# yandooo/cilium

Hardware: AMD Instinct MI355X
Metric: L7 verdicts/sec + scanned GB/s (HBM roofline frac), 1/2/4/8 MI355X (higher is better)
Workload: dtype u8

## Files before the change

### cilium_amd/csrc/capi.cc

```cpp
#include <algorithm>
#include <cstring>

#include "engine/nfa_pool.h"
#include "engine_state.h"
#include "policy/npds_proto.h"
#include "regex/nfa_walk.h"
#include "regex/re_dfa.h"

namespace {

void set_err(char *err, size_t errlen, const std::string &m) {
    if (!err || errlen == 0) return;
    size_t n = std::min(errlen - 1, m.size());
    memcpy(err, m.data(), n);
    err[n] = 0;
}

template <class T>
size_t Put(std::vector<uint8_t> &blob, const std::vector<T> &v) {
    size_t off = (blob.size() + 255) & ~(size_t)255;
    blob.resize(off + v.size() * sizeof(T) + 16);
    if (!v.empty()) memcpy(blob.data() + off, v.data(), v.size() * sizeof(T));
    return off;
}
// ... 246 lines not shown
    e->mc = std::make_unique<McCompiler>(e->ps.get());
    e->r2 = std::make_unique<R2Compiler>(e->ps.get());
    e->cs = std::make_unique<CassCompiler>(e->ps.get());
    return e;
}

void l7g_engine_destroy(l7g_engine *e) {
    if (!e) return;
    if (e->device < 0) { delete e; return; }
    hipSetDevice(e->device);
    StopServices(e);
    hipDeviceSynchronize();
    if (e->d_blob) hipFree(e->d_blob);
    if (e->d_conns) hipFree(e->d_conns);
    e->hctx.clear();
    e->scr.clear();
    if (e->d_flow) hipFree(e->d_flow);
    if (e->d_zreg) hipFree(e->d_zreg);
    if (e->zreg_ev) hipEventDestroy(e->zreg_ev);
    for (hipEvent_t ev : e->prof_ev)
        if (ev) hipEventDestroy(ev);
    delete e;
}

int l7g_policy_update(l7g_engine *e, const char *json, size_t len, char *err, size_t errlen) {
    return l7g_policy_update_view(e, (const uint8_t *)json, len, 0, 0, err, errlen);
}

int l7g_policy_update_proto(l7g_engine *e, const uint8_t *buf, size_t len, char *err, size_t errlen) {
    return l7g_policy_update_view(e, buf, len, 1, 0, err, errlen);
}

constexpr uint64_t kTablesMagic = 0x3154473754L;
constexpr uint64_t kTablesAbi = 2ull << 56 | (uint64_t)sizeof(DevRuleset) << 48 | (uint64_t)sizeof(DevNfa) << 36 |
                                (uint64_t)sizeof(ImgHeader) << 24 | (uint64_t)sizeof(DevKafkaRuleset) << 12 |
                                (uint64_t)sizeof(McImgHeader);

int l7g_tables_export(l7g_engine *e, uint8_t *buf, size_t cap, size_t *len) {
    std::lock_guard<std::mutex> g(e->mu);
    Ser s;
    s.u64(kTablesMagic);
    s.u64(kTablesAbi);
    s.u64((uint64_t)e->policy_form);
    s.u64((uint64_t)e->policy_px);
    s.str(e->policy_src);
    e->hc->Save(s);
    e->kc->Save(s);
    e->mc->Save(s);
    e->r2->Save(s);
    e->cs->Save(s);
    if (len) *len = s.out.size();
    if (!buf || cap < s.out.size()) return -2;
    memcpy(buf, s.out.data(), s.out.size());
    return 0;
}

int l7g_tables_import(l7g_engine *e, const uint8_t *buf, size_t len, char *err, size_t errlen) {
    std::lock_guard<std::mutex> g(e->mu);
    Des d(buf, len);
    if (d.u64() != kTablesMagic) { set_err(err, errlen, "not an l7g_tables_export image"); return -1; }
    if (d.u64() != kTablesAbi) { set_err(err, errlen, "tables image from a build with another table layout"); return -1; }
    const int form = (int)d.u64(), px = (int)d.u64();
    const std::string src = d.str();
    if (!d.ok) { set_err(err, errlen, "truncated tables image"); return -1; }
    auto ps = std::make_unique<PolicySet>();
    std::string m;
    const bool ok = form ? LoadPolicySetProto((const uint8_t *)src.data(), src.size(), ps.get(), &m)
// ... 218 lines not shown
```

### cilium_amd/csrc/device_tables.h

```cpp
#pragma once
#include <stddef.h>
#include <stdint.h>

#if defined(__HIPCC__)
#define L7_HD __host__ __device__
#else
#define L7_HD
#endif

namespace l7 {

enum : uint8_t {
    V_DENY = 0, V_ALLOW = 1, V_PARSE_ERROR = 2, V_INCOMPLETE = 3, V_UNSUPPORTED = 4,
};
enum : uint8_t { PROTO_NONE = 0, PROTO_HTTP = 1, PROTO_KAFKA = 2, PROTO_MEMCACHE = 3, PROTO_R2D2 = 4, PROTO_CASSANDRA = 5 };
#define L7_PROTO_OWNED(p) ((p) >= PROTO_HTTP && (p) <= PROTO_CASSANDRA)

#ifndef L7_KAFKA_CLASSES
#define L7_KAFKA_CLASSES 8
#endif

constexpr int kCntWords = 32;
constexpr int kCntMc = L7_KAFKA_CLASSES;
constexpr int kCntHttp = L7_KAFKA_CLASSES + 2;
// ... 55 lines not shown
    uint16_t len;
    uint16_t pad;
    uint32_t name_off;
};
struct ImgHeader {
    uint8_t nchunks;
    uint8_t nhdr;
    uint8_t terminal;
    uint8_t ndfa;
    uint8_t slot_dfa[kNumSlots + 1];
    uint8_t max_slot_dfas;
    uint8_t pad0[3];
    uint16_t ref_slots;
    uint16_t pad1;
    uint32_t dfa_off;
    uint32_t init_off;
    uint32_t absent_off;
    uint32_t rule_off;
    uint32_t hdr_off;
    uint32_t total_states;
    uint32_t name_cls_off;
    uint32_t name_trans_off;
    uint32_t name_info_off;
    uint16_t name_ncls;
    uint16_t name_states;
    uint32_t nfa_off;
    uint8_t nnfa;
    uint8_t ntab_bits;
    uint8_t pad2[2];
    uint32_t ntab_off;
    uint32_t ntab_mul;
};
static_assert(sizeof(ImgHeader) == 80, "ImgHeader layout");

struct DevNameEnt {
    uint32_t w[4];
    uint8_t len;
    uint8_t info;
    uint8_t pad[10];
};
L7_HD inline uint32_t l7_name_hash(uint32_t w0, uint32_t w1, uint32_t w2, uint32_t w3, uint32_t len, uint32_t mul,
                                   uint32_t bits) {
    uint32_t x = w0 ^ (w1 * 0x85EBCA6Bu) ^ (w2 * 0xC2B2AE35u) ^ (w3 * 0x27D4EB2Fu) ^ len;
    x ^= x >> 15;
    return (x * mul) >> (32 - bits);
}

constexpr int kNfaMaxWords = 16;
constexpr int kNfaMaxPositions = 1 << 20;
struct DevNfaSparse {
    uint64_t row_of_off;
    uint64_t row_ptr_off;
    uint64_t pair_w_off;
    uint64_t pair_m_off;
};
struct DevNfa {
    uint32_t m, W, K, nivl;
    uint64_t t_off;
    uint64_t ivl_off;
    uint64_t b_off;
    uint64_t acc_off;
    uint64_t ascii_off;
    uint8_t condmap[64];
};
constexpr int kMaxNfaPerRuleset = 64;
struct DevNfaRef {
// ... 176 lines not shown
```

### cilium_amd/csrc/engine/http_compile.cc

```cpp
#include "http_compile.h"

#include <algorithm>
#include <cstring>
#include <functional>
#include <memory>

#include "../regex/re_dfa.h"
#include "nfa_pool.h"

namespace l7 {

namespace {

constexpr int kSlotNever = 0xFF;
int FixedSlot(const std::string &name) {
    if (name == ":method") return SLOT_METHOD;
    if (name == ":path") return SLOT_PATH;
    if (name == ":authority") return SLOT_AUTHORITY;
    if (name == "host" || name == "x-envoy-original-dst-host") return kSlotNever;
    if (!name.empty() && name[0] == ':') return kSlotNever;
    return -1;
}

struct Pat {
// ... 377 lines not shown
                    if (rp.second == nf.pat && (a == 1) == pats[rp.second].invert) m[rp.first >> 6] &= ~bit(rp.first);
            }
        }
        H.max_slot_dfas = (uint8_t)std::max<size_t>(H.max_slot_dfas, dfas.size());
        for (size_t g = 0; g < dfas.size(); g++) {
            Built b{slot, std::move(dfas[g]), {}, 0};
            b.absorb = SortAbsorbing(b.d);
            const std::vector<int> &sub = groups[g];
            std::vector<int> local(pats.size(), -1);
            for (size_t q = 0; q < sub.size(); q++) local[sub[q]] = (int)q;
            b.masks.resize((size_t)b.d.nstates * nchunks);
            for (int s = 0; s < b.d.nstates; s++) {
                uint64_t *m = &b.masks[(size_t)s * nchunks];
                for (size_t c = 0; c < nchunks; c++) m[c] = all[c];
                for (auto &rp : rm_pat) {
                    int q = local[rp.second];
                    if (q < 0) continue;
                    bool acc = (b.d.accept[s][q >> 6] >> (q & 63)) & 1;
                    if (acc == pats[rp.second].invert) m[rp.first >> 6] &= ~bit(rp.first);
                }
            }
            built.push_back(std::move(b));
        }
    }
    if (built.size() > 255) { *err = "rule set needs more than 255 DFAs"; return -1; }
    if (nfas.size() > (size_t)kMaxNfaPerRuleset) { *err = "rule set needs more than 64 NFA matchers"; return -1; }
    H.nnfa = (uint8_t)nfas.size();
    H.ndfa = (uint8_t)built.size();
    for (int s = 0, k = 0; s <= kNumSlots; s++) {
        while (k < (int)built.size() && built[k].slot < s) k++;
        H.slot_dfa[s] = (uint8_t)k;
    }

    std::vector<uint8_t> img(sizeof(ImgHeader));
    std::vector<DevDfa> dd(built.size());
    H.dfa_off = Append(img, dd.data(), dd.size());
    H.init_off = Append(img, init.data(), init.size());
    H.absent_off = Append(img, absent.data(), absent.size());
    std::vector<int32_t> ids(nchunks * 64, -1);
    for (size_t r = 0; r < nr; r++) ids[r] = rules[r]->id;
    H.rule_off = Append(img, ids.data(), ids.size());
    std::vector<DevHdrName> hn;
    std::vector<uint8_t> names;
    for (auto &nm : custom) {
        DevHdrName h{};
        uint32_t hash = kFnvBasis;
        for (char c : nm) hash = l7_fnv_step(hash, (uint8_t)c);
        h.hash = hash;
        h.len = (uint16_t)nm.size();
        h.name_off = (uint32_t)names.size();
        names.insert(names.end(), nm.begin(), nm.end());
        hn.push_back(h);
    }
    {
        std::vector<DevNfaRef> refs(nfas.size());
        for (size_t k = 0; k < nfas.size(); k++) {
            refs[k].nfa = nfas[k].nfa;
            refs[k].slot = (uint8_t)nfas[k].slot;
            refs[k].mask_off = Append(img, nfas[k].masks.data(), nfas[k].masks.size());
        }
        H.nfa_off = Append(img, refs.data(), refs.size());
    }
    H.hdr_off = Append(img, hn.data(), hn.size());
    uint32_t names_off = Append(img, names.data(), names.size());
    for (auto &h : hn) h.name_off += names_off;
    if (!hn.empty()) memcpy(img.data() + H.hdr_off, hn.data(), hn.size() * sizeof(DevHdrName));
    {
        NameDfa nd = BuildNameDfa(custom);
        H.name_ncls = (uint16_t)nd.ncls;
        H.name_states = (uint16_t)nd.info.size();
        H.name_cls_off = Append(img, nd.cls, 256);
        H.name_trans_off = Append(img, nd.trans.data(), nd.trans.size());
        H.name_info_off = Append(img, nd.info.data(), nd.info.size());
        uint32_t bits = 0, mul = 0;
        const std::vector<DevNameEnt> tab = BuildNameTable(custom, &bits, &mul);
        H.ntab_bits = (uint8_t)bits;
        H.ntab_mul = mul;
        H.ntab_off = Append(img, tab.data(), tab.size());
    }
    for (size_t k = 0; k < built.size(); k++) {
        const re::DFA &d = built[k].d;
        dd[k].ncls = (uint16_t)d.ncls;
        dd[k].start = (uint16_t)d.start;
        dd[k].cls_off = Append(img, d.cls, 256);
        dd[k].trans_off = Append(img, d.next.data(), d.next.size());
        dd[k].mask_off = Append(img, built[k].masks.data(), built[k].masks.size());
        dd[k].absorb = built[k].absorb;
        H.total_states += (uint32_t)d.nstates;
    }
    memcpy(img.data() + H.dfa_off, dd.data(), dd.size() * sizeof(DevDfa));
    memcpy(img.data(), &H, sizeof H);
    img.resize((img.size() + 15) & ~(size_t)15);

    HttpImage &I = img_;
    DevRuleset rs{};
    rs.image_off = (uint32_t)I.images.size();
    rs.image_len = (uint32_t)img.size();
    if ((uint64_t)rs.image_off + img.size() > 0xFFFFFFFFull) { *err = "HTTP rule tables exceed 4 GiB"; return -1; }
    I.images.insert(I.images.end(), img.begin(), img.end());
    I.rulesets.push_back(rs);
    I.chunks += nchunks;
    I.dfas += built.size();
    I.dfa_states += H.total_states;
    return (int)I.rulesets.size() - 1;
}

}
```

### cilium_amd/csrc/kernels/http_classify.hip

```cpp
#include <hip/hip_runtime.h>

#include <algorithm>
#include <cstddef>

#include "../device_tables.h"
#include "copy_in.h"
#include "gmem.h"
#include "launch.h"
#include "service.h"

extern "C" __device__ __attribute__((const)) unsigned long long __ockl_wfred_min_u64(unsigned long long);
extern "C" __device__ __attribute__((const)) unsigned long long __ockl_wfred_max_u64(unsigned long long);
extern "C" __device__ __attribute__((const)) unsigned long long __ockl_wfred_and_u64(unsigned long long);

namespace l7 {

namespace {

constexpr int kWaves = 8;
constexpr int kBlock = 64 * kWaves;
constexpr uint32_t kWin = 256;
constexpr uint32_t kWinChunks = kWin / 16;
constexpr uint32_t kWaveLds = 64 * kWin;
constexpr uint32_t kOffImg = kWaves * kWaveLds;
// ... 11 lines not shown
#define PH_DECL uint64_t ph_t = __builtin_amdgcn_s_memtime(); uint64_t ph_acc[8] = {0, 0, 0, 0, 0, 0, 0, 0};
#define PH_MARK(slot) do { const uint64_t ph_n = __builtin_amdgcn_s_memtime(); ph_acc[slot] += ph_n - ph_t; ph_t = ph_n; } while (0)
#define PH_COUNT(slot, v) (ph_acc[slot] += (v))
#define PH_FLUSH(lane) do { if ((lane) == 0) for (int ph_i = 0; ph_i < 8; ph_i++) atomicAdd(&g_phase[ph_i], (unsigned long long)ph_acc[ph_i]); } while (0)
#else
#define PH_DECL
#define PH_MARK(slot) do {} while (0)
#define PH_COUNT(slot, v) do {} while (0)
#define PH_FLUSH(lane) do {} while (0)
#endif
#ifdef L7G_PHASE_TIMING
#define LAT_T0 uint64_t lat_t = __builtin_amdgcn_s_memtime();
#define LAT_T(slot) do { const uint64_t lat_n = __builtin_amdgcn_s_memtime(); if ((threadIdx.x & 63) == 0) atomicAdd(&g_phase[slot], (unsigned long long)(lat_n - lat_t)); lat_t = lat_n; } while (0)
#define LAT_N(slot) do { if ((threadIdx.x & 63) == 0) atomicAdd(&g_phase[slot], 1ull); } while (0)
#else
#define LAT_T0
#define LAT_T(slot) do {} while (0)
#define LAT_N(slot) do {} while (0)
#endif

enum : uint32_t {
    M_METHOD, M_TARGET, M_VERSION, M_LINE, M_NAME, M_OWS, M_VALUE, M_SKIP, M_LF, M_ENDLF, M_DONE,
    M_CHSIZE, M_CHEXT, M_CHLF, M_CHDATA, M_CHDCR, M_CHDLF, M_TRL, M_TRLSCAN, M_TRLLF, M_TRLEND
};
constexpr uint32_t kNoSlot = 0xFF;

__constant__ uint32_t kVer[10] = {'H', 'T', 'T', 'P', '/', 0x100, '.', 0x100, '\r', '\n'};

__device__ __forceinline__ bool is_tchar(uint32_t c) {
    const uint32_t m1 = 0x03FF6CFAu;
    const uint32_t m2 = 0xC7FFFFFEu;
    const uint32_t m3 = 0x57FFFFFFu;
    const uint32_t w = c < 0x40 ? m1 : (c < 0x60 ? m2 : m3);
    return (c - 0x20u < 0x60u) && ((w >> (c & 31)) & 1);
}

__device__ __forceinline__ uint32_t stop_bits(uint32_t x) {
    const uint32_t t = x & 0x7F7F7F7Fu;
    return (~(t + 0x60606060u) | (t + 0x01010101u)) & ~x & 0x80808080u;
}
__device__ __forceinline__ uint32_t nib(uint32_t s) { return __builtin_amdgcn_ubfe((s >> 7) * 0x204081u, 21, 4); }
__device__ __forceinline__ uint32_t stop_mask(uint4 w) {
    return nib(stop_bits(w.x)) | nib(stop_bits(w.y)) << 4 | nib(stop_bits(w.z)) << 8 | nib(stop_bits(w.w)) << 12;
}
__device__ __forceinline__ uint32_t tstop_bits(uint32_t x) {
    const uint32_t t = x & 0x7F7F7F7Fu;
    return (~(t + 0x5F5F5F5Fu) | (t + 0x01010101u)) & ~x & 0x80808080u;
}
__device__ __forceinline__ uint32_t vstop_bits(uint32_t x) {
    const uint32_t t = x ^ 0x09090909u;
    const uint32_t ht = ~(((t & 0x7F7F7F7Fu) + 0x7F7F7F7Fu) | t) & 0x80808080u;
    return stop_bits(x) & ~ht;
}
__device__ __forceinline__ uint32_t stop_any(uint4 w) {
    const uint32_t a = w.x & 0x7F7F7F7Fu, b = w.y & 0x7F7F7F7Fu, c = w.z & 0x7F7F7F7Fu, d = w.w & 0x7F7F7F7Fu;
    const uint32_t s = ((~(a + 0x60606060u) | (a + 0x01010101u)) & ~w.x) | ((~(b + 0x60606060u) | (b + 0x01010101u)) & ~w.y) |
                       ((~(c + 0x60606060u) | (c + 0x01010101u)) & ~w.z) | ((~(d + 0x60606060u) | (d + 0x01010101u)) & ~w.w);
    return s & 0x80808080u;
}
__device__ __forceinline__ uint32_t alnum_bits(uint32_t x) {
    const uint32_t h = x | 0x80808080u;
    const uint32_t l = x | 0xA0A0A0A0u;
    const uint32_t dig = (h - 0x30303030u) & ~(h - 0x3A3A3A3Au);
    const uint32_t let = (l - 0x61616161u) & ~(l - 0x7B7B7B7Bu);
    const uint32_t t = x ^ 0x2D2D2D2Du;
    const uint32_t dash = ~(((t & 0x7F7F7F7Fu) + 0x7F7F7F7Fu) | t);
    return (dig | let | dash) & ~x & 0x80808080u;
}
// ... 23 lines not shown
    __device__ __forceinline__ uint4 u128(uint32_t o) const { return *(const uint4 *)(p + o); }
};
template <bool kLds>
__device__ __forceinline__ uint32_t uni(uint32_t v) {
    return kLds ? (uint32_t)__builtin_amdgcn_readfirstlane((int)v) : v;
}
#define HDR_U32(I, field) uni<kLds>((I).u32(offsetof(ImgHeader, field)))
#define HDR_U16(I, field) uni<kLds>((I).u16(offsetof(ImgHeader, field)))
#define HDR_U8(I, field) uni<kLds>((I).u8(offsetof(ImgHeader, field)))

struct Lane {
    uint64_t base;
    uint32_t a0;
    uint32_t lena;
    uint32_t pa;
    uint32_t w;
    uint32_t mode;
    uint32_t mark;
    uint32_t idx;
    bool done;
    bool owed;
    bool scan;
    bool tail;
    uint8_t verdict;
    int32_t rule;
    uint32_t consumed;
    uint32_t present;
    uint32_t slot;
    uint32_t nstate;
    uint32_t ninfo;
    bool have_cl, chunked, cl_bad, cl_ws, in_ows;
    uint32_t ndig;
    uint64_t clv, cl;
    uint32_t dcls, dtrans, dmask, dncls, st, saved;
    uint32_t dabs;
    uint64_t acc[kChunksPerPass];
    uint32_t cg, dg;
};
static_assert(kDfasPerPass == 1, "one DFA per slot per framing pass");

template <bool kLds>
__device__ __forceinline__ void slot_begin(const Img<kLds> &I, Lane &L, uint32_t slot) {
    const uint32_t lo = I.u8(offsetof(ImgHeader, slot_dfa) + slot) + L.dg;
    const uint32_t hi = I.u8(offsetof(ImgHeader, slot_dfa) + slot + 1);
    L.st = 0;
    L.dcls = L.dtrans = L.dmask = L.dncls = L.dabs = 0;
    if (lo < hi) {
        const uint32_t d = HDR_U32(I, dfa_off) + lo * sizeof(DevDfa);
        L.dcls = I.u32(d + 0);
        L.dtrans = I.u32(d + 4);
        L.dmask = I.u32(d + 8);
        const uint32_t nc_st = I.u32(d + 12);
        L.dncls = nc_st & 0xFFFF;
        L.st = nc_st >> 16;
        L.dabs = I.u32(d + 16);
    }
}

template <bool kLds>
__device__ __forceinline__ void dfa_step(const Img<kLds> &I, Lane &L, uint32_t c) {
    if (L.st) L.st = I.u16(L.dtrans + 2 * (L.st * L.dncls + I.u8(L.dcls + c)));
}

template <bool kLds>
__device__ __forceinline__ void slot_end(const Img<kLds> &I, Lane &L) {
    if (L.dtrans == 0) return;
    const uint32_t nchunks = HDR_U8(I, nchunks);
    const uint32_t nc = nchunks > L.cg ? min(nchunks - L.cg, (uint32_t)kChunksPerPass) : 0;
    const uint32_t base = L.dmask + 8 * (L.st * nchunks + L.cg);
#pragma unroll
    for (int c = 0; c < kChunksPerPass; c++)
        if ((uint32_t)c < nc) L.acc[c] &= I.u64(base + 8 * c);
}

template <bool kLds>
__device__ __forceinline__ void acc_init(const Img<kLds> &I, Lane &L) {
    const uint32_t nchunks = HDR_U8(I, nchunks);
#pragma unroll
    for (int c = 0; c < kChunksPerPass; c++)
        L.acc[c] = L.cg + c < nchunks ? I.u64(HDR_U32(I, init_off) + 8 * (L.cg + c)) : 0;
}

template <bool kLds>
__device__ __forceinline__ void frame_reset(const Img<kLds> &I, Lane &L) {
    L.pa = L.a0;
    L.mode = M_METHOD;
    L.mark = L.a0;
    L.present = 0;
    L.have_cl = L.chunked = false;
    L.cl = 0;
    slot_begin(I, L, SLOT_METHOD);
}

__device__ __forceinline__ void finish(Lane &L, uint8_t v, int32_t rule = -1) {
    L.done = true;
    L.scan = false;
    L.mode = M_DONE;
    L.verdict = v;
    L.rule = rule;
// ... 64 lines not shown
            } else {
                verdict_then_body(L, (uint8_t)HDR_U8(I, terminal), -1);
            }
        }
    }
}

template <bool kLds>
__device__ __forceinline__ bool line_done(const Img<kLds> &I, Lane &L) {
    bool ok = true;
    if (L.ninfo & NI_CL) {
        ok = !(L.have_cl || L.ndig == 0 || L.ndig > 10 || L.cl_bad);
        L.have_cl = true;
        L.cl = L.clv;
    }
    if ((L.ninfo & NI_TE) && L.ndig == 7) L.chunked = true;
    if (L.slot != kNoSlot) {
        slot_end(I, L);
        L.present |= 1u << L.slot;
    }
    return ok;
}

struct Cursor {
    const uint8_t *slot;
    uint32_t swz;
    uint32_t w;
    __device__ __forceinline__ uint4 chunk(uint32_t k) const {
        return *(const uint4 *)(slot + (((k << 4) & (kWin - 16)) ^ swz));
    }
    __device__ __forceinline__ uint32_t at(uint32_t p) const { return slot[((p - w) & (kWin - 1)) ^ swz]; }
};

template <int kKind>
__device__ __forceinline__ uint32_t find_stop(const Cursor &C, uint32_t pa, uint32_t lim) {
    while (pa < lim) {
        const uint4 w = C.chunk((pa - C.w) >> 4);
        uint32_t m = (kKind == 0 ? tstop_mask(w) : kKind == 1 ? vstop_mask(w) : nonalnum_mask(w)) & (0xFFFFu << (pa & 15));
        const uint32_t cend = (pa & ~15u) + 16;
        if (cend > lim) m &= (1u << (lim & 15)) - 1u;
        if (m) return (pa & ~15u) + (uint32_t)__builtin_ctz(m);
        pa = cend;
    }
    return lim;
}

template <bool kLds>
__device__ __forceinline__ void ows_done(const Img<kLds> &I, Lane &L) {
    if (L.slot == kNoSlot && !(L.ninfo & (NI_CL | NI_TE))) {
        L.mode = M_SKIP;
    } else {
        L.mode = M_VALUE;
        if (L.slot != kNoSlot) {
            slot_begin(I, L, L.slot);
        } else {
            L.st = 0;
            L.dcls = L.dtrans = 0;
        }
        L.in_ows = false;
        L.clv = 0;
        L.ndig = 0;
        L.cl_bad = L.cl_ws = false;
    }
}

template <bool kLds>
__device__ __forceinline__ void name_slot(const Img<kLds> &I, Lane &L) {
    uint32_t s = kNoSlot;
    if (L.ninfo & NI_HOST) s = SLOT_AUTHORITY;
    else if (L.ninfo & NI_CUSTOM) s = SLOT_CUSTOM0 + (L.ninfo & NI_CUSTOM) - 1;
    if (s != kNoSlot && ((L.present >> s) & 1)) s = kNoSlot;
    if (s != kNoSlot && !((HDR_U32(I, ref_slots) >> s) & 1)) s = kNoSlot;
    L.slot = s;
}

__device__ __forceinline__ uint32_t ws_mask(uint4 w) {
    auto eq = [](uint32_t x, uint32_t b) {
        const uint32_t t = x ^ b;
        return ~(((t & 0x7F7F7F7Fu) + 0x7F7F7F7Fu) | t) & 0x80808080u;
    };
    return nib(eq(w.x, 0x20202020u) | eq(w.x, 0x09090909u)) | nib(eq(w.y, 0x20202020u) | eq(w.y, 0x09090909u)) << 4 |
           nib(eq(w.z, 0x20202020u) | eq(w.z, 0x09090909u)) << 8 | nib(eq(w.w, 0x20202020u) | eq(w.w, 0x09090909u)) << 12;
}

template <bool kLds>
__device__ __forceinline__ void fast_line(const Img<kLds> &I, Lane &L, const Cursor &C, const uint64_t *nfa_bits) {
    const uint32_t k0 = (L.pa - C.w) >> 4, o = L.pa & 15, i = o >> 2, sh = (o & 3) * 8;
    const uint4 a = C.chunk(k0), b = C.chunk(k0 + 1);
    const uint32_t d1 = i == 0 ? a.y : i == 1 ? a.z : i == 2 ? a.w : b.x;
    const uint32_t d0 = i == 0 ? a.x : i == 1 ? a.y : i == 2 ? a.z : a.w;
// ... 21 lines not shown
    if (nb == 0) return;
    auto keep = [e](uint32_t j) { return e >= 4 * j + 4 ? 0xFFFFFFFFu : e <= 4 * j ? 0u : (1u << (8 * (e - 4 * j))) - 1u; };
    const uint32_t w0 = (f.x | 0x20202020u) & keep(0), w1 = (f.y | 0x20202020u) & keep(1);
    const uint32_t w2 = (f.z | 0x20202020u) & keep(2), w3 = (f.w | 0x20202020u) & keep(3);
    const uint32_t h = l7_name_hash(w0, w1, w2, w3, e, HDR_U32(I, ntab_mul), nb);
    const uint32_t ent = HDR_U32(I, ntab_off) + h * (uint32_t)sizeof(DevNameEnt);
    const uint4 n = I.u128(ent);
    const uint32_t meta = I.u32(ent + 16);
    const bool hit = (meta & 0xFF) == e && n.x == w0 && n.y == w1 && n.z == w2 && n.w == w3;
    L.mark = L.pa;
    L.ninfo = hit ? (meta >> 8) & 0xFF : 0u;
    name_slot(I, L);
    const uint32_t v = (uint32_t)__builtin_ctz((~ws_mask(f) & (0xFFFFu << (e + 1)) & 0xFFFFu) | 0x10000u);
    if (v < 16) {
        L.pa += v;
        ows_done(I, L);
    } else {
        L.pa += e + 1;
        L.mode = M_OWS;
    }
}

template <bool kLds>
__device__ __forceinline__ void parse_window(const Img<kLds> &I, Lane &L, Cursor &C, const uint64_t *nfa_bits) {
    const uint32_t lim = min(L.w + kWin, L.lena);
    C.w = L.w;
    const uint32_t ncls_name = HDR_U16(I, name_ncls);
    const uint32_t name_cls = HDR_U32(I, name_cls_off), name_trans = HDR_U32(I, name_trans_off);

    if (L.mode == M_METHOD) {
        uint32_t c = 0;
        if (L.pa < lim) {
            c = C.at(L.pa);
            uint32_t k = L.dcls ? I.u8(L.dcls + c) : 0;
            uint32_t c1 = L.pa + 1 < lim ? C.at(L.pa + 1) : 0;
            while (is_tchar(c)) {
                const uint32_t p1 = L.pa + 1;
                const uint32_t c2 = p1 + 1 < lim ? C.at(p1 + 1) : 0;
                const uint32_t k1 = L.dcls ? I.u8(L.dcls + c1) : 0;
                if (L.st) L.st = I.u16(L.dtrans + 2 * (L.st * L.dncls + k));
                L.pa = p1;
                if (p1 >= lim) break;
                c = c1;
                c1 = c2;
                k = k1;
            }
        }
        if (L.pa < lim) {
            if (c != ' ' || L.pa == L.mark) {
                finish(L, V_PARSE_ERROR);
            } else {
                slot_end(I, L);
                L.present |= 1u << SLOT_METHOD;
                L.pa++;
                L.mark = L.pa;
                L.mode = M_TARGET;
                slot_begin(I, L, SLOT_PATH);
            }
        }
    }
    if (L.mode == M_TARGET) {
        uint32_t c = 0;
        if (L.pa < lim) {
            c = C.at(L.pa);
            uint32_t k = L.dcls ? I.u8(L.dcls + c) : 0;
            uint32_t c1 = L.pa + 1 < lim ? C.at(L.pa + 1) : 0;
            while (c > 0x20 && c != 0x7F && L.st != 0 && L.st < L.dabs) {
                const uint32_t p1 = L.pa + 1;
                const uint32_t c2 = p1 + 1 < lim ? C.at(p1 + 1) : 0;
                const uint32_t k1 = L.dcls ? I.u8(L.dcls + c1) : 0;
                if (L.st) L.st = I.u16(L.dtrans + 2 * (L.st * L.dncls + k));
                L.pa = p1;
                if (p1 >= lim) break;
                c = c1;
                c1 = c2;
                k = k1;
            }
        }
        if (L.pa < lim && c > 0x20 && c != 0x7F) {
            L.pa = find_stop<0>(C, L.pa, lim);
            c = L.pa < lim ? C.at(L.pa) : 0;
        }
        if (L.pa < lim) {
            if (c != ' ' || L.pa == L.mark) {
                finish(L, V_PARSE_ERROR);
            } else {
                slot_end(I, L);
                L.present |= 1u << SLOT_PATH;
                L.pa++;
                L.mark = 0;
                L.mode = M_VERSION;
            }
        }
    }
    if (L.mode == M_VERSION) {
        if (L.mark == 0 && L.pa + 10 <= lim) {
            const uint32_t k0 = (L.pa - L.w) >> 4, o = L.pa & 15, i = o >> 2, sh = o & 3;
            const uint4 a = C.chunk(k0), b = C.chunk(k0 + 1);
            const uint32_t e0 = i == 0 ? a.x : i == 1 ? a.y : i == 2 ? a.z : a.w;
            const uint32_t e1 = i == 0 ? a.y : i == 1 ? a.z : i == 2 ? a.w : b.x;
            const uint32_t e2 = i == 0 ? a.z : i == 1 ? a.w : i == 2 ? b.x : b.y;
            const uint32_t e3 = i == 0 ? a.w : i == 1 ? b.x : i == 2 ? b.y : b.z;
            const uint32_t r0 = __builtin_amdgcn_alignbyte(e1, e0, sh);
            const uint32_t r1 = __builtin_amdgcn_alignbyte(e2, e1, sh);
            const uint32_t r2 = __builtin_amdgcn_alignbyte(e3, e2, sh);
            if (r0 == 0x50545448u && (r1 & 0x00FF00FFu) == 0x002E002Fu && ((r1 >> 8) & 0xFF) - '0' < 10u &&
                (r1 >> 24) - '0' < 10u && (r2 & 0xFFFFu) == 0x0A0Du) {
                L.pa += 10;
                L.mark = 10;
// ... 2 lines not shown
        for (; L.pa < lim && L.mark < 10; L.pa++, L.mark++) {
            const uint32_t c = C.at(L.pa);
            const uint32_t want = kVer[L.mark];
            if (want == 0x100 ? c - '0' >= 10u : c != want) break;
        }
        if (L.mark == 10) L.mode = M_LINE;
        else if (L.pa < lim) finish(L, V_PARSE_ERROR);
    }
    while (L.mode >= M_LINE && L.mode < M_DONE && L.pa < lim) {
        if (L.mode == M_LINE && L.pa + 16 <= lim) fast_line(I, L, C, nfa_bits);
        if (L.mode == M_LINE) {
            if (C.at(L.pa) == '\r') {
                L.pa++;
                L.mode = M_ENDLF;
            } else {
                L.mode = M_NAME;
                L.mark = L.pa;
                L.nstate = kNameStart;
            }
        }
        if (L.mode == M_ENDLF && L.pa < lim) {
            if (C.at(L.pa) != '\n') {
                finish(L, V_PARSE_ERROR);
            } else {
                L.pa++;
                headers_done(I, L, nfa_bits);
            }
        }
        if (L.mode == M_NAME) {
            uint32_t c = 0;
            if (L.pa < lim) {
                c = C.at(L.pa);
                uint32_t k = I.u8(name_cls + c);
                uint32_t c1 = L.pa + 1 < lim ? C.at(L.pa + 1) : 0;
                while (k != 0 && L.nstate != kNameOther) {
                    const uint32_t p1 = L.pa + 1;
                    const uint32_t c2 = p1 + 1 < lim ? C.at(p1 + 1) : 0;
                    const uint32_t k1 = I.u8(name_cls + c1);
                    L.nstate = I.u16(name_trans + 2 * (L.nstate * ncls_name + k));
                    L.pa = p1;
                    if (p1 >= lim) break;
                    c = c1;
                    c1 = c2;
                    k = k1;
                }
                if (L.pa < lim && k != 0) {
                    L.pa = find_stop<2>(C, L.pa, lim);
                    c = L.pa < lim ? C.at(L.pa) : 0;
                    while (L.pa < lim && c != ':' && is_tchar(c)) {
                        L.pa++;
                        c = L.pa < lim ? C.at(L.pa) : 0;
                    }
                }
            }
            if (L.pa < lim) {
                if (c != ':' || L.pa == L.mark) {
                    finish(L, V_PARSE_ERROR);
                } else {
                    L.pa++;
                    L.ninfo = L.nstate >= kNameStart ? I.u8(HDR_U32(I, name_info_off) + L.nstate) : 0;
                    name_slot(I, L);
                    L.mode = M_OWS;
                }
            }
        }
        if (L.mode == M_OWS) {
            for (; L.pa < lim; L.pa++) {
                const uint32_t c = C.at(L.pa);
                if (c != ' ' && c != '\t') break;
            }
            if (L.pa < lim) ows_done(I, L);
        }
        if (L.mode == M_VALUE && !(L.ninfo & (NI_CL | NI_TE))) {
            uint32_t c = 0, nx = 0;
            if (L.pa < lim) {
                c = C.at(L.pa);
                uint32_t k = L.dcls ? I.u8(L.dcls + c) : 0;
                uint32_t c1 = L.pa + 1 < lim ? C.at(L.pa + 1) : 0;
                while (!((c < 0x20 && c != '\t') || c == 0x7F) && (L.in_ows || (L.st != 0 && L.st < L.dabs))) {
                    const uint32_t p1 = L.pa + 1;
                    const uint32_t c2 = p1 + 1 < lim ? C.at(p1 + 1) : 0;
                    const uint32_t k1 = L.dcls ? I.u8(L.dcls + c1) : 0;
                    const bool ws = c == ' ' || c == '\t';
                    if (ws && !L.in_ows) L.saved = L.st;
                    L.in_ows = ws;
                    if (L.st) L.st = I.u16(L.dtrans + 2 * (L.st * L.dncls + k));
                    L.pa = p1;
                    if (p1 >= lim) break;
                    c = c1;
                    c1 = c2;
                    k = k1;
                }
                if (L.pa + 1 < lim) nx = c1 | 0x100;
            }
            if (L.pa < lim && !((c < 0x20 && c != '\t') || c == 0x7F)) {
                L.pa = find_stop<1>(C, L.pa, lim);
                c = L.pa < lim ? C.at(L.pa) : 0;
                nx = 0;
            }
            if (L.pa < lim) {
                if (c != '\r') {
                    finish(L, V_PARSE_ERROR);
                } else {
                    if (L.in_ows) L.st = L.saved;
                    if (nx) {
                        L.pa += 2;
                        if (nx != ('\n' | 0x100)) finish(L, V_PARSE_ERROR);
                        else if (line_done(I, L)) L.mode = M_LINE;
                        else finish(L, V_PARSE_ERROR);
                    } else {
                        L.pa++;
                        L.mode = M_LF;
                    }
                }
            }
        }
        if (L.mode == M_VALUE) {
            uint32_t c = 0;
            const bool te = (L.ninfo & NI_TE) != 0;
            for (; L.pa < lim; L.pa++) {
                c = C.at(L.pa);
                if ((c < 0x20 && c != '\t') || c == 0x7F) break;
                const bool ws = c == ' ' || c == '\t';
                if (ws && !L.in_ows) L.saved = L.st;
// ... 229 lines not shown
            const uint32_t j = jb + s;
            wait_vmcnt<kRing - 1>();
            if (j < npieces) {
                uint4 v;
                asm volatile("ds_read_b128 %0, %1\n\ts_waitcnt lgkmcnt(0)"
                             : "=v"(v)
                             : "v"((uint32_t)(uintptr_t)(wave_lds + s * 1024 + 16 * lane))
                             : "memory");
                const bool ok = (j << 6) + lane < vtot;
                const uint64_t M = __ballot(ok && stop_any(v) != 0);
                const uint32_t q = j - j0;
#pragma unroll
                for (int t = 0; t < 4; t++)
                    if (q == (uint32_t)t) {
                        pc[2 * t] = (uint32_t)M;
                        pc[2 * t + 1] = (uint32_t)(M >> 32);
                    }
            }
            MAP_PIECE(s, j + kRing);
        }
    }
    wait_vmcnt<0>();
#undef MAP_PIECE
    const uint32_t sh = vs & 63, wsh = sh >> 5, bsh = sh & 31;
#pragma unroll
    for (int w = 0; w < (int)kMapWords; w++) {
        const uint32_t a0 = wsh ? pc[w + 1] : pc[w];
        const uint32_t a1 = wsh ? (w + 2 < 8 ? pc[w + 2] : 0u) : pc[w + 1];
        T.m[w] = __builtin_amdgcn_alignbit(a1, a0, bsh);
    }
    T.off = 0;
}

__device__ __forceinline__ bool build_tile_map(TileMap &T, Lane &L, uint32_t lane, uint8_t *wave_lds) {
#pragma unroll
    for (int q = 0; q < (int)kMapWords; q++) T.m[q] = 0;
    T.off = kMapChunks;
    T.from = 0;
    const uint32_t nch = min(map_nch(L), kMapChunks);
    const uint32_t nseg = (nch + 3) >> 2;
    const uint32_t smax = (uint32_t)__builtin_amdgcn_readfirstlane((int)__ockl_wfred_max_u32(nseg));
    if (smax == 0) return false;
    const uint64_t act = __ballot(nch > 0);
    const uint64_t dummy = (uint64_t)__shfl((unsigned long long)L.base, (int)__builtin_ctzll(act));
    asm volatile("s_waitcnt lgkmcnt(0)" ::: "memory");
    {
        uint64_t lo = __ockl_wfred_min_u64(nch ? L.base : ~0ull);
        uint64_t hi = __ockl_wfred_max_u64(nch ? L.base + ((uint64_t)nch << 4) : 0ull);
        uint32_t own = __ockl_wfred_add_u32(nch);
        lo = ((uint64_t)(uint32_t)__builtin_amdgcn_readfirstlane((int)(uint32_t)(lo >> 32)) << 32) |
             (uint32_t)__builtin_amdgcn_readfirstlane((int)(uint32_t)lo);
        hi = ((uint64_t)(uint32_t)__builtin_amdgcn_readfirstlane((int)(uint32_t)(hi >> 32)) << 32) |
             (uint32_t)__builtin_amdgcn_readfirstlane((int)(uint32_t)hi);
        own = (uint32_t)__builtin_amdgcn_readfirstlane((int)own);
        const uint64_t span = (hi - lo) >> 4;
        if (span <= kSpanChunksMax && span <= (uint64_t)own + (own >> 3)) {
            map_span(T, L, lane, wave_lds, lo, (uint32_t)span, nch);
            return false;
        }
    }
    T.off = kMapChunks - 4 * smax;
    T.from = 4 * kSkipSteps;
    if (smax <= kSkipSteps) return false;
    {
        dma_windows_issue(wave_lds, window_packed(L), lane);
        const uint32_t smax8 = (smax + 1) >> 1, skip8 = kWin / 128;
        T.off = kMapChunks - 8 * smax8;
        const uint32_t sub8 = lane & 7, grp8 = lane >> 3;
        uint64_t qb8[8];
        uint32_t qn8[8];
#pragma unroll
        for (int q = 0; q < 8; q++) {
            qb8[q] = (uint64_t)__shfl((unsigned long long)L.base, 8 * q + (int)grp8);
            qn8[q] = (uint32_t)__shfl((int)nch, 8 * q + (int)grp8);
        }
        constexpr int kMapDepth = 3;
        gm_u32x4 buf[kMapDepth][8];
#define MAP_LOAD8(s, j)                                                                                        \
    do {                                                                                                       \
        _Pragma("unroll") for (int q_ = 0; q_ < 8; q_++) {                                                     \
            const uint32_t c_ = 8 * (uint32_t)(j) + sub8;                                                      \
            const uint64_t a_ = c_ < qn8[q_] ? qb8[q_] + ((uint64_t)c_ << 4) : dummy;                          \
            asm volatile("global_load_dwordx4 %0, %1, off" : "=v"(buf[s][q_]) : "v"(a_) : "memory");           \
        }                                                                                                      \
    } while (0)
#pragma unroll
        for (int s = 0; s < kMapDepth; s++) MAP_LOAD8(s, skip8 + (uint32_t)s);
        for (uint32_t j0 = skip8; j0 < smax8; j0 += kMapDepth) {
#pragma unroll
            for (int s = 0; s < kMapDepth; s++) {
                const uint32_t j = j0 + s;
                asm volatile("s_waitcnt vmcnt(%8)"
                             : "+v"(buf[s][0]), "+v"(buf[s][1]), "+v"(buf[s][2]), "+v"(buf[s][3]), "+v"(buf[s][4]),
                               "+v"(buf[s][5]), "+v"(buf[s][6]), "+v"(buf[s][7])
                             : "n"(8 * (kMapDepth - 1)));
                uint64_t M[8];
#pragma unroll
                for (int q = 0; q < 8; q++) M[q] = __ballot(stop_any(u4(buf[s][q])) != 0);
                MAP_LOAD8(s, j + kMapDepth);
                if (j < smax8) {
                    const uint32_t qo = lane >> 3;
                    uint64_t Mq = M[0];
#pragma unroll
                    for (int q = 1; q < 8; q++) Mq = qo == (uint32_t)q ? M[q] : Mq;
                    uint32_t nb = (uint32_t)(Mq >> (8 * (lane & 7))) & 0xFFu;
                    if (8 * j >= nch) nb = 0;
#pragma unroll
                    for (int q = 0; q < (int)kMapWords - 1; q++) T.m[q] = __builtin_amdgcn_alignbit(T.m[q + 1], T.m[q], 8);
                    T.m[kMapWords - 1] = (T.m[kMapWords - 1] >> 8) | (nb << 24);
// ... 61 lines not shown
        if (L.pa >= L.lena) {
            L.pa = L.lena;
            finish(L, V_INCOMPLETE);
            return;
        }
    }
}

template <bool kLds>
__device__ __forceinline__ void finish_tail(const Img<kLds> &I, Lane &L, const uint64_t *nfa_bits) {
    L.tail = false;
    L.pa += 4;
    if (line_done(I, L)) {
        L.mode = M_LINE;
        headers_done(I, L, nfa_bits);
    } else {
        finish(L, V_PARSE_ERROR);
    }
}

struct Out {
    uint8_t *verdict;
    int32_t *rule;
    uint32_t *consumed;
    const uint64_t *nfa_bits;
};

__device__ __forceinline__ void emit(const Lane &L, const Out &O) {
    O.verdict[L.idx] = L.verdict;
    O.rule[L.idx] = L.rule;
    O.consumed[L.idx] = L.consumed;
}

template <bool kLds, bool kFlush = true, bool kInit = true>
__device__ __forceinline__ void run_tile(Lane &L, const uint8_t *img, uint8_t *wave_lds, uint32_t lane, const Out &O,
                                         const TileMap *pre = nullptr) {
    const Img<kLds> I{img};
    L.scan = false;
    L.tail = false;
    if (kInit && !L.done) {
        L.cg = 0;
        L.dg = 0;
        acc_init(I, L);
        frame_reset(I, L);
        if (L.lena == L.a0) finish(L, V_INCOMPLETE);
    }
    PH_DECL
    TileMap TM;
    bool loaded = false;
    if (pre) TM = *pre;
    else loaded = build_tile_map(TM, L, lane, wave_lds);
    PH_MARK(2);
    Cursor C;
    C.slot = wave_lds + lane * kWin;
    C.swz = win_swizzle(lane) << 4;
    while (__any(!L.done)) {
        const uint64_t packed = window_packed(L);
        PH_MARK(3);
        if (!loaded) dma_windows(wave_lds, packed, lane);
        loaded = false;
        PH_MARK(0);
        if (!L.done) {
            parse_window(I, L, C, O.nfa_bits);
            if (!L.done && !L.scan && L.pa >= L.lena) finish(L, V_INCOMPLETE);
        }
        PH_MARK(1);
        PH_COUNT(5, __builtin_popcountll(__ballot(L.scan)));
        map_skip(L, TM);
        if (L.tail) finish_tail(I, L, O.nfa_bits);
        PH_MARK(2);
        if (L.done && L.owed) {
            emit(L, O);
            L.owed = false;
        }
        PH_COUNT(4, 1);
    }
    if (L.done && L.owed) {
        emit(L, O);
        L.owed = false;
    }
    PH_MARK(3);
    PH_COUNT(6, 1);
    if (kFlush) PH_FLUSH(lane);
}


__device__ __forceinline__ uint32_t cr_mask(uint4 w) {
    auto eq = [](uint32_t x) {
        const uint32_t t = x ^ 0x0D0D0D0Du;
        return ~(((t & 0x7F7F7F7Fu) + 0x7F7F7F7Fu) | t) & 0x80808080u;
    };
    return nib(eq(w.x)) | nib(eq(w.y)) << 4 | nib(eq(w.z)) << 8 | nib(eq(w.w)) << 12;
}

constexpr uint32_t kLatLines = 63;

template <bool kLds>
__device__ __forceinline__ void lat_request(const Lane &L, const uint8_t *img, uint8_t *wave_lds, uint32_t lane,
                                            const Out &O) {
    const Img<kLds> I{img};
    const uint32_t a0 = L.a0, lena = L.lena;
    if (lena == a0) {
        if (lane == 0) {
            Lane W = L;
            finish(W, V_INCOMPLETE);
            emit(W, O);
        }
        return;
    }
    LAT_T0
    const uint32_t nch = (lena + 15) >> 4;
    uint32_t *crpos = reinterpret_cast<uint32_t *>(wave_lds);
    const uint64_t below = (1ull << lane) - 1;
    uint32_t ncr = 0;
    int hend = -1;
    bool all = false;
    TileMap TM;
#pragma unroll
    for (int q = 0; q < (int)kMapWords; q++) TM.m[q] = 0;
    TM.off = 0;
    TM.from = 0;
    constexpr uint32_t kLfKnown = 1u << 31, kLfYes = 1u << 30, kPos = kLfYes - 1;
    for (uint32_t c0 = 0;; c0 += 64) {
        const uint32_t c = c0 + lane;
        uint32_t m = 0;
        uint4 w = make_uint4(0, 0, 0, 0);
        if (c < nch) {
// ... 21 lines not shown
        for (uint32_t r = ncr + ex; m; m &= m - 1, r++) {
            const uint32_t b = (uint32_t)__builtin_ctz(m);
            const bool known = b < 15 || (lane < 63 && c + 1 < nch);
            const uint32_t nx = b < 15 ? byte_of(w, b + 1) : nb0;
            if (r < kLatLines + 2) crpos[r] = (16 * c + b) | (known ? kLfKnown : 0u) | (known && nx == '\n' ? kLfYes : 0u);
        }
        ncr += tot;
        __builtin_amdgcn_fence(__ATOMIC_RELEASE, "wavefront");
        __builtin_amdgcn_wave_barrier();
        __builtin_amdgcn_fence(__ATOMIC_ACQUIRE, "wavefront");
        const uint32_t have = min(ncr, kLatLines + 1);
        const uint64_t eb =
            __ballot(lane >= 1 && lane < have && (crpos[lane] & kPos) == (crpos[lane - 1] & kPos) + 2);
        if (eb) {
            hend = (int)__builtin_ctzll(eb);
            break;
        }
        if (c0 + 64 >= nch) {
            all = true;
            break;
        }
        if (ncr > kLatLines) break;
    }
    LAT_T(9);
    if (!(hend > 0 || (all && ncr <= kLatLines))) {
        asm volatile("s_waitcnt lgkmcnt(0)" ::: "memory");
        Lane W = L;
        if (lane != 0) {
            W.done = true;
            W.owed = false;
            W.base = 0;
            W.a0 = W.pa = W.lena = 0;
        }
        run_tile<kLds>(W, img, wave_lds, lane, O);
        return;
    }
    uint32_t nl;
    if (hend > 0) {
        nl = (uint32_t)hend;
    } else {
        const uint32_t sp = ncr ? (crpos[ncr - 1] & kPos) + 2 : a0;
        nl = ncr + (sp < lena ? 1u : 0u);
    }
    uint32_t start = a0, cr = 0;
    const bool has_cr = lane < nl && lane < ncr;
    if (lane < nl && lane > 0) start = (crpos[lane - 1] & kPos) + 2;
    if (has_cr) cr = crpos[lane] & kPos;
    const uint32_t lend = has_cr ? min(cr + 2, lena) : lena;
    const bool act = lane < nl && start < lend;
    const uint32_t cr_end_w = hend > 0 ? crpos[hend] : 0u, cr_end = cr_end_w & kPos;
    asm volatile("s_waitcnt lgkmcnt(0)" ::: "memory");
    __builtin_amdgcn_wave_barrier();
    const bool complete = has_cr && cr + 2 <= lena;
    Lane W = L;
    W.owed = false;
    W.cg = 0;
    W.dg = 0;
    acc_init(I, W);
    frame_reset(I, W);
    if (act) {
        W.lena = lend;
        if (lane > 0) {
#pragma unroll
            for (int c = 0; c < kChunksPerPass; c++) W.acc[c] = ~0ull;
            W.pa = W.mark = start;
            W.mode = M_LINE;
            W.st = 0;
            W.dcls = W.dtrans = W.dmask = W.dncls = W.dabs = 0;
            W.slot = kNoSlot;
        }
    } else {
        W.done = true;
        W.base = 0;
        W.a0 = W.pa = W.lena = 0;
    }
    run_tile<kLds, true, false>(W, img, wave_lds, lane, O, &TM);
    LAT_T(10);
    const bool bad = act && W.verdict == V_PARSE_ERROR;
    const bool inc = act && !bad && !complete;
    const uint64_t clb = __ballot(act && W.have_cl);
    const bool err = __ballot(bad) != 0 || __popcll(clb) > 1;
    const bool any_inc = __ballot(inc) != 0;
    const uint64_t cl = clb ? (uint64_t)__shfl((unsigned long long)W.cl, (int)__builtin_ctzll(clb)) : 0ull;
    const bool chunked = __ballot(act && W.chunked) != 0;
    const uint32_t pres = act ? W.present : 0u;
    bool keep = act;
#pragma unroll
    for (int sl = 0; sl < 16; sl++) {
        const bool mine = lane >= 1 && act && pres == (1u << sl);
        const uint64_t mk = __ballot(mine);
        if (mine && lane != (uint32_t)__builtin_ctzll(mk)) keep = false;
    }
    const uint32_t present = __ockl_wfred_or_u32(keep ? pres : 0u);
    uint64_t acc[kChunksPerPass];
#pragma unroll
    for (int c = 0; c < kChunksPerPass; c++) acc[c] = __ockl_wfred_and_u64(keep ? W.acc[c] : ~0ull);
    if (lane != 0) {
        W.done = true;
        W.owed = false;
        W.base = 0;
        W.a0 = W.pa = W.lena = 0;
    } else {
        W.done = false;
        W.owed = true;
        W.scan = W.tail = false;
        W.lena = lena;
        if (err) {
            finish(W, V_PARSE_ERROR);
        } else if (hend <= 0 || any_inc || cr_end + 1 >= lena) {
            finish(W, V_INCOMPLETE);
        } else if ((cr_end_w & kLfKnown) ? !(cr_end_w & kLfYes) : *(const uint8_t *)(L.base + cr_end + 1) != '\n') {
            finish(W, V_PARSE_ERROR);
        } else {
            W.pa = cr_end + 2;
            W.mode = M_LINE;
            W.present = present;
#pragma unroll
            for (int c = 0; c < kChunksPerPass; c++) W.acc[c] = acc[c];
            W.have_cl = clb != 0;
            W.cl = cl;
            W.chunked = chunked;
            headers_done(I, W, O.nfa_bits);
        }
    }
    if (__ballot(lane == 0 && !W.done)) run_tile<kLds, true, false>(W, img, wave_lds, lane, O);
    else if (lane == 0) emit(W, O);
    LAT_T(11);
}

constexpr uint32_t kFastMaxChunks = 256;
constexpr uint32_t kFastOffCr = kFastMaxChunks * 16, kFastOffLf = kFastOffCr + 2 * kFastMaxChunks;
constexpr uint32_t kFastOffBad = kFastOffLf + 2 * kFastMaxChunks, kFastOffPos = kFastOffBad + 2 * kFastMaxChunks;
static_assert(kFastOffPos + 4 * 64 <= kWaveLds, "fast path LDS layout");

__device__ __forceinline__ uint32_t byte_mask(uint4 w, uint32_t b) {
    const uint32_t bb = b * 0x01010101u;
    auto eq = [bb](uint32_t x) {
        const uint32_t t = x ^ bb;
        return ~(((t & 0x7F7F7F7Fu) + 0x7F7F7F7Fu) | t) & 0x80808080u;
    };
    return nib(eq(w.x)) | nib(eq(w.y)) << 4 | nib(eq(w.z)) << 8 | nib(eq(w.w)) << 12;
}
__device__ __forceinline__ uint32_t fast_bad_mask(uint4 w) {
    return stop_mask(w) & ~(byte_mask(w, '\t') | byte_mask(w, '\r') | byte_mask(w, '\n'));
}

template <bool kLds>
__device__ __forceinline__ bool lat_fast(const Lane &L, const uint8_t *img, uint8_t *wave_lds, uint32_t lane,
                                         const Out &O) {
    const Img<kLds> I{img};
    LAT_T0
    const uint32_t a0 = L.a0, lena = L.lena;
    const uint32_t nch = (lena + 15) >> 4;
    const uint32_t nchunks = HDR_U8(I, nchunks);
    if (lena <= a0 || nch > kFastMaxChunks || HDR_U8(I, nnfa) != 0 || HDR_U8(I, max_slot_dfas) > 1 ||
        nchunks > (uint32_t)kChunksPerPass || HDR_U8(I, ntab_bits) == 0)
        return false;
    uint16_t *crm = reinterpret_cast<uint16_t *>(wave_lds + kFastOffCr);
// ... 596 lines not shown
```

Baseline: 2.875 billion.

## Use null DFA sentinel and branchless LDS walk loops in HTTP classifier

Reserves a zeroed 256-byte null DFA region after the image header so lanes without a DFA can step unconditionally through state 0, which removes the per-byte `if (st)` and `dcls ?` checks. The compiler now rejects DFAs whose dead state transitions elsewhere. The byte walk loops are rewritten as branchless steps that issue the transition, class and next-byte LDS reads together in inline asm, and row stride multiplication uses umul24. Separately, the latency-path tile map prefetch depth is reduced from 3 to 2 through a new template parameter. The risks are dropping the explicit bounds checks on lookahead reads, which now rely on the window contents, and bumping the tables ABI version.

```diff
diff --git a/cilium_amd/csrc/capi.cc b/cilium_amd/csrc/capi.cc
--- a/cilium_amd/csrc/capi.cc
+++ b/cilium_amd/csrc/capi.cc
@@ -302,7 +302,7 @@
 }
 
 constexpr uint64_t kTablesMagic = 0x3154473754L;
-constexpr uint64_t kTablesAbi = 2ull << 56 | (uint64_t)sizeof(DevRuleset) << 48 | (uint64_t)sizeof(DevNfa) << 36 |
+constexpr uint64_t kTablesAbi = 3ull << 56 | (uint64_t)sizeof(DevRuleset) << 48 | (uint64_t)sizeof(DevNfa) << 36 |
                                 (uint64_t)sizeof(ImgHeader) << 24 | (uint64_t)sizeof(DevKafkaRuleset) << 12 |
                                 (uint64_t)sizeof(McImgHeader);
 
diff --git a/cilium_amd/csrc/device_tables.h b/cilium_amd/csrc/device_tables.h
--- a/cilium_amd/csrc/device_tables.h
+++ b/cilium_amd/csrc/device_tables.h
@@ -111,6 +111,8 @@
     uint32_t ntab_mul;
 };
 static_assert(sizeof(ImgHeader) == 80, "ImgHeader layout");
+constexpr uint32_t kImgNullDfaOff = sizeof(ImgHeader);
+constexpr uint32_t kImgNullDfaBytes = 256;
 
 struct DevNameEnt {
     uint32_t w[4];
diff --git a/cilium_amd/csrc/engine/http_compile.cc b/cilium_amd/csrc/engine/http_compile.cc
--- a/cilium_amd/csrc/engine/http_compile.cc
+++ b/cilium_amd/csrc/engine/http_compile.cc
@@ -433,7 +433,7 @@
         H.slot_dfa[s] = (uint8_t)k;
     }
 
-    std::vector<uint8_t> img(sizeof(ImgHeader));
+    std::vector<uint8_t> img(kImgNullDfaOff + kImgNullDfaBytes);
     std::vector<DevDfa> dd(built.size());
     H.dfa_off = Append(img, dd.data(), dd.size());
     H.init_off = Append(img, init.data(), init.size());
@@ -481,6 +481,8 @@
     }
     for (size_t k = 0; k < built.size(); k++) {
         const re::DFA &d = built[k].d;
+        for (int c = 0; c < d.ncls; c++)
+            if (d.next[c] != 0) { *err = "DFA whose dead state is left again"; return -1; }
         dd[k].ncls = (uint16_t)d.ncls;
         dd[k].start = (uint16_t)d.start;
         dd[k].cls_off = Append(img, d.cls, 256);
diff --git a/cilium_amd/csrc/kernels/http_classify.hip b/cilium_amd/csrc/kernels/http_classify.hip
--- a/cilium_amd/csrc/kernels/http_classify.hip
+++ b/cilium_amd/csrc/kernels/http_classify.hip
@@ -67,8 +67,10 @@
     const uint32_t m2 = 0xC7FFFFFEu;
     const uint32_t m3 = 0x57FFFFFFu;
     const uint32_t w = c < 0x40 ? m1 : (c < 0x60 ? m2 : m3);
-    return (c - 0x20u < 0x60u) && ((w >> (c & 31)) & 1);
-}
+    return (c - 0x20u < 0x60u) & ((w >> (c & 31)) & 1);
+}
+
+__device__ __forceinline__ bool value_stop(uint32_t c) { return ((c < 0x20) & (c != '\t')) | (c == 0x7F); }
 
 __device__ __forceinline__ uint32_t stop_bits(uint32_t x) {
     const uint32_t t = x & 0x7F7F7F7Fu;
@@ -158,39 +160,49 @@
     bool have_cl, chunked, cl_bad, cl_ws, in_ows;
     uint32_t ndig;
     uint64_t clv, cl;
-    uint32_t dcls, dtrans, dmask, dncls, st, saved;
-    uint32_t dabs;
+    uint32_t dcls, dtrans, dmask, drow, st, saved;
+    uint32_t dabs1;
     uint64_t acc[kChunksPerPass];
     uint32_t cg, dg;
 };
 static_assert(kDfasPerPass == 1, "one DFA per slot per framing pass");
 
+__device__ __forceinline__ void null_dfa(Lane &L) {
+    L.st = 0;
+    L.dcls = L.dtrans = kImgNullDfaOff;
+    L.dmask = L.drow = 0;
+    L.dabs1 = ~0u;
+}
+
 template <bool kLds>
 __device__ __forceinline__ void slot_begin(const Img<kLds> &I, Lane &L, uint32_t slot) {
     const uint32_t lo = I.u8(offsetof(ImgHeader, slot_dfa) + slot) + L.dg;
     const uint32_t hi = I.u8(offsetof(ImgHeader, slot_dfa) + slot + 1);
-    L.st = 0;
-    L.dcls = L.dtrans = L.dmask = L.dncls = L.dabs = 0;
+    null_dfa(L);
     if (lo < hi) {
         const uint32_t d = HDR_U32(I, dfa_off) + lo * sizeof(DevDfa);
         L.dcls = I.u32(d + 0);
         L.dtrans = I.u32(d + 4);
         L.dmask = I.u32(d + 8);
         const uint32_t nc_st = I.u32(d + 12);
-        L.dncls = nc_st & 0xFFFF;
+        L.drow = 2 * (nc_st & 0xFFFF);
         L.st = nc_st >> 16;
-        L.dabs = I.u32(d + 16);
-    }
-}
-
+        L.dabs1 = I.u32(d + 16) - 1;
+    }
+}
+
+__device__ __forceinline__ uint32_t row_addr(uint32_t trans, uint32_t st, uint32_t row, uint32_t k) {
+    return __umul24(st, row) + (trans + 2 * k);
+}
 template <bool kLds>
 __device__ __forceinline__ void dfa_step(const Img<kLds> &I, Lane &L, uint32_t c) {
-    if (L.st) L.st = I.u16(L.dtrans + 2 * (L.st * L.dncls + I.u8(L.dcls + c)));
-}
+    L.st = I.u16(row_addr(L.dtrans, L.st, L.drow, I.u8(L.dcls + c)));
+}
+__device__ __forceinline__ bool walk_live(const Lane &L) { return L.st - 1u < L.dabs1; }
 
 template <bool kLds>
 __device__ __forceinline__ void slot_end(const Img<kLds> &I, Lane &L) {
-    if (L.dtrans == 0) return;
+    if (L.dmask == 0) return;
     const uint32_t nchunks = HDR_U8(I, nchunks);
     const uint32_t nc = nchunks > L.cg ? min(nchunks - L.cg, (uint32_t)kChunksPerPass) : 0;
     const uint32_t base = L.dmask + 8 * (L.st * nchunks + L.cg);
@@ -321,6 +333,28 @@
     __device__ __forceinline__ uint32_t at(uint32_t p) const { return slot[((p - w) & (kWin - 1)) ^ swz]; }
 };
 
+template <bool kLds>
+__device__ __forceinline__ void walk_step(const Img<kLds> &I, const Cursor &C, uint32_t trans, uint32_t row, uint32_t cls,
+                                          uint32_t &st, uint32_t &k, uint32_t c1, uint32_t p2, uint32_t &c2) {
+    const uint32_t ta = row_addr(trans, st, row, k);
+    if constexpr (kLds) {
+        const uint32_t ib = (uint32_t)(uintptr_t)I.p;
+        const uint32_t ba = (uint32_t)(uintptr_t)C.slot + (((p2 - C.w) & (kWin - 1)) ^ C.swz);
+        uint32_t s_ = ib + ta, k_ = ib + cls + c1, c_ = ba;
+        asm volatile("ds_read_u16 %0, %0\n\tds_read_u8 %1, %1\n\tds_read_u8 %2, %2\n\ts_waitcnt lgkmcnt(0)"
+                     : "+v"(s_), "+v"(k_), "+v"(c_)
+                     :
+                     : "memory");
+        st = s_;
+        k = k_;
+        c2 = c_;
+    } else {
+        st = I.u16(ta);
+        k = I.u8(cls + c1);
+        c2 = C.at(p2);
+    }
+}
+
 template <int kKind>
 __device__ __forceinline__ uint32_t find_stop(const Cursor &C, uint32_t pa, uint32_t lim) {
     while (pa < lim) {
@@ -343,8 +377,7 @@
         if (L.slot != kNoSlot) {
             slot_begin(I, L, L.slot);
         } else {
-            L.st = 0;
-            L.dcls = L.dtrans = 0;
+            null_dfa(L);
         }
         L.in_ows = false;
         L.clv = 0;
@@ -432,18 +465,16 @@
         uint32_t c = 0;
         if (L.pa < lim) {
             c = C.at(L.pa);
-            uint32_t k = L.dcls ? I.u8(L.dcls + c) : 0;
-            uint32_t c1 = L.pa + 1 < lim ? C.at(L.pa + 1) : 0;
-            while (is_tchar(c)) {
-                const uint32_t p1 = L.pa + 1;
-                const uint32_t c2 = p1 + 1 < lim ? C.at(p1 + 1) : 0;
-                const uint32_t k1 = L.dcls ? I.u8(L.dcls + c1) : 0;
-                if (L.st) L.st = I.u16(L.dtrans + 2 * (L.st * L.dncls + k));
-                L.pa = p1;
-                if (p1 >= lim) break;
+            uint32_t k = I.u8(L.dcls + c);
+            uint32_t c1 = C.at(L.pa + 1);
+            bool go = is_tchar(c);
+            while (go) {
+                uint32_t c2;
+                walk_step(I, C, L.dtrans, L.drow, L.dcls, L.st, k, c1, L.pa + 2, c2);
+                L.pa++;
                 c = c1;
                 c1 = c2;
-                k = k1;
+                go = (L.pa < lim) & is_tchar(c);
             }
         }
         if (L.pa < lim) {
@@ -463,18 +494,16 @@
         uint32_t c = 0;
         if (L.pa < lim) {
             c = C.at(L.pa);
-            uint32_t k = L.dcls ? I.u8(L.dcls + c) : 0;
-            uint32_t c1 = L.pa + 1 < lim ? C.at(L.pa + 1) : 0;
-            while (c > 0x20 && c != 0x7F && L.st != 0 && L.st < L.dabs) {
-                const uint32_t p1 = L.pa + 1;
-                const uint32_t c2 = p1 + 1 < lim ? C.at(p1 + 1) : 0;
-                const uint32_t k1 = L.dcls ? I.u8(L.dcls + c1) : 0;
-                if (L.st) L.st = I.u16(L.dtrans + 2 * (L.st * L.dncls + k));
-                L.pa = p1;
-                if (p1 >= lim) break;
+            uint32_t k = I.u8(L.dcls + c);
+            uint32_t c1 = C.at(L.pa + 1);
+            bool go = (c > 0x20) & (c != 0x7F) & walk_live(L);
+            while (go) {
+                uint32_t c2;
+                walk_step(I, C, L.dtrans, L.drow, L.dcls, L.st, k, c1, L.pa + 2, c2);
+                L.pa++;
                 c = c1;
                 c1 = c2;
-                k = k1;
+                go = (L.pa < lim) & (c > 0x20) & (c != 0x7F) & walk_live(L);
             }
         }
         if (L.pa < lim && c > 0x20 && c != 0x7F) {
@@ -543,17 +572,15 @@
             if (L.pa < lim) {
                 c = C.at(L.pa);
                 uint32_t k = I.u8(name_cls + c);
-                uint32_t c1 = L.pa + 1 < lim ? C.at(L.pa + 1) : 0;
-                while (k != 0 && L.nstate != kNameOther) {
-                    const uint32_t p1 = L.pa + 1;
-                    const uint32_t c2 = p1 + 1 < lim ? C.at(p1 + 1) : 0;
-                    const uint32_t k1 = I.u8(name_cls + c1);
-                    L.nstate = I.u16(name_trans + 2 * (L.nstate * ncls_name + k));
-                    L.pa = p1;
-                    if (p1 >= lim) break;
+                uint32_t c1 = C.at(L.pa + 1);
+                bool go = (k != 0) & (L.nstate != kNameOther);
+                while (go) {
+                    uint32_t c2;
+                    walk_step(I, C, name_trans, 2 * ncls_name, name_cls, L.nstate, k, c1, L.pa + 2, c2);
+                    L.pa++;
                     c = c1;
                     c1 = c2;
-                    k = k1;
+                    go = (L.pa < lim) & (k != 0) & (L.nstate != kNameOther);
                 }
                 if (L.pa < lim && k != 0) {
                     L.pa = find_stop<2>(C, L.pa, lim);
@@ -586,21 +613,19 @@
             uint32_t c = 0, nx = 0;
             if (L.pa < lim) {
                 c = C.at(L.pa);
-                uint32_t k = L.dcls ? I.u8(L.dcls + c) : 0;
-                uint32_t c1 = L.pa + 1 < lim ? C.at(L.pa + 1) : 0;
-                while (!((c < 0x20 && c != '\t') || c == 0x7F) && (L.in_ows || (L.st != 0 && L.st < L.dabs))) {
-                    const uint32_t p1 = L.pa + 1;
-                    const uint32_t c2 = p1 + 1 < lim ? C.at(p1 + 1) : 0;
-                    const uint32_t k1 = L.dcls ? I.u8(L.dcls + c1) : 0;
-                    const bool ws = c == ' ' || c == '\t';
-                    if (ws && !L.in_ows) L.saved = L.st;
+                uint32_t k = I.u8(L.dcls + c);
+                uint32_t c1 = C.at(L.pa + 1);
+                bool go = !value_stop(c) & (L.in_ows | walk_live(L));
+                while (go) {
+                    const bool ws = (c == ' ') | (c == '\t');
+                    L.saved = (ws & !L.in_ows) ? L.st : L.saved;
                     L.in_ows = ws;
-                    if (L.st) L.st = I.u16(L.dtrans + 2 * (L.st * L.dncls + k));
-                    L.pa = p1;
-                    if (p1 >= lim) break;
+                    uint32_t c2;
+                    walk_step(I, C, L.dtrans, L.drow, L.dcls, L.st, k, c1, L.pa + 2, c2);
+                    L.pa++;
                     c = c1;
                     c1 = c2;
-                    k = k1;
+                    go = (L.pa < lim) & !value_stop(c) & (L.in_ows | walk_live(L));
                 }
                 if (L.pa + 1 < lim) nx = c1 | 0x100;
             }
@@ -896,6 +921,7 @@
     T.off = 0;
 }
 
+template <int kMapDepth>
 __device__ __forceinline__ bool build_tile_map(TileMap &T, Lane &L, uint32_t lane, uint8_t *wave_lds) {
 #pragma unroll
     for (int q = 0; q < (int)kMapWords; q++) T.m[q] = 0;
@@ -938,7 +964,6 @@
             qb8[q] = (uint64_t)__shfl((unsigned long long)L.base, 8 * q + (int)grp8);
             qn8[q] = (uint32_t)__shfl((int)nch, 8 * q + (int)grp8);
         }
-        constexpr int kMapDepth = 3;
         gm_u32x4 buf[kMapDepth][8];
 #define MAP_LOAD8(s, j)                                                                                        \
     do {                                                                                                       \
@@ -1066,7 +1091,7 @@
     O.consumed[L.idx] = L.consumed;
 }
 
-template <bool kLds, bool kFlush = true, bool kInit = true>
+template <bool kLds, bool kFlush = true, bool kInit = true, int kMapDepth = 3>
 __device__ __forceinline__ void run_tile(Lane &L, const uint8_t *img, uint8_t *wave_lds, uint32_t lane, const Out &O,
                                          const TileMap *pre = nullptr) {
     const Img<kLds> I{img};
@@ -1083,7 +1108,7 @@
     TileMap TM;
     bool loaded = false;
     if (pre) TM = *pre;
-    else loaded = build_tile_map(TM, L, lane, wave_lds);
+    else loaded = build_tile_map<kMapDepth>(TM, L, lane, wave_lds);
     PH_MARK(2);
     Cursor C;
     C.slot = wave_lds + lane * kWin;
@@ -1127,6 +1152,7 @@
     return nib(eq(w.x)) | nib(eq(w.y)) << 4 | nib(eq(w.z)) << 8 | nib(eq(w.w)) << 12;
 }
 
+constexpr int kLatMapDepth = 2;
 constexpr uint32_t kLatLines = 63;
 
 template <bool kLds>
@@ -1214,7 +1240,7 @@
             W.base = 0;
             W.a0 = W.pa = W.lena = 0;
         }
-        run_tile<kLds>(W, img, wave_lds, lane, O);
+        run_tile<kLds, true, true, kLatMapDepth>(W, img, wave_lds, lane, O);
         return;
     }
     uint32_t nl;
@@ -1247,8 +1273,7 @@
             for (int c = 0; c < kChunksPerPass; c++) W.acc[c] = ~0ull;
             W.pa = W.mark = start;
             W.mode = M_LINE;
-            W.st = 0;
-            W.dcls = W.dtrans = W.dmask = W.dncls = W.dabs = 0;
+            null_dfa(W);
             W.slot = kNoSlot;
         }
     } else {
@@ -1256,7 +1281,7 @@
         W.base = 0;
         W.a0 = W.pa = W.lena = 0;
     }
-    run_tile<kLds, true, false>(W, img, wave_lds, lane, O, &TM);
+    run_tile<kLds, true, false, kLatMapDepth>(W, img, wave_lds, lane, O, &TM);
     LAT_T(10);
     const bool bad = act && W.verdict == V_PARSE_ERROR;
     const bool inc = act && !bad && !complete;
@@ -1305,7 +1330,7 @@
             headers_done(I, W, O.nfa_bits);
         }
     }
-    if (__ballot(lane == 0 && !W.done)) run_tile<kLds, true, false>(W, img, wave_lds, lane, O);
+    if (__ballot(lane == 0 && !W.done)) run_tile<kLds, true, false, kLatMapDepth>(W, img, wave_lds, lane, O);
     else if (lane == 0) emit(W, O);
     LAT_T(11);
 }
```

Result: faster. 2.942 billion, median of 6 (+2.3%).
